# fcastagna/JoXSZ

Hardware: AMD Instinct MI355X
Metric: walker-likelihoods/sec at 512^2 map, 500-pt grid (higher is better)
Workload: dtype f64; 1 GPU; 1024 walkers/GPU, 512x512 SZ map, 500-pt radial grid, joint X-ray+SZ likelihood, synthetic CL J1226.9+3332-shaped inputs (BASELINE configs[2]); walkers_per_gpu=1024, S=512, N=500, B=55, chunk=1024, route=map, conv=custom, form=exact, sampling=none, radial_sampling=none, truncation=none, parallelism=walkers sharded x1, device=AMD GPU (gfx950:sramecc+:xnack-, 256 CUs)

## Files before the change

### joxsz_amd/csrc/joxsz_hip.hip

```cpp
#include <dlfcn.h>
#include <unistd.h>

#include <cctype>

#include "jx_ctx.hpp"

static int g_rocfft_refs = 0;

static size_t tensor_bytes(const jx_config& c, int id) {
    const size_t f = sizeof(double);
    switch (id) {
        case JX_T_R_PP: return f * c.N;
        case JX_T_D_MAT: return f * (size_t)c.S * c.S;
        case JX_T_BEAM_2D: return f * (size_t)c.B * c.B;
        case JX_T_FILTERING: return f * (size_t)c.S * c.S;
        case JX_T_RADIUS: return f * c.S;
        case JX_T_FLUX_DATA: return f * 3 * c.nflux;
        case JX_T_CONV_T: case JX_T_CONV_V: return f * c.nconv;
        case JX_T_PAR_VALS: case JX_T_PAR_MIN: case JX_T_PAR_MAX: case JX_T_PAR_MU: case JX_T_PAR_SIGMA:
            return f * c.npar;
        case JX_T_PAR_KIND: return sizeof(int32_t) * c.npar;
        case JX_T_THAWED_IDX: return sizeof(int32_t) * c.ndim;
        case JX_T_X_R_NE: case JX_T_X_R_T: case JX_T_GEOMAREA: return f * c.nann;
        case JX_T_PROJVOLS: return f * (size_t)c.nann * c.nann;
// ... 71 lines not shown
    if (d.quad) {
        d.pairw = 2;
        if (map_lds_need(d, threads) > (LDS_MAX - 2048) / 2) d.pairw = 1;
    } else if (pair_full && d.fast_map) {
        d.pairw = 2;
        if (map_lds_need(d, threads) > LDS_MAX - 1024) d.pairw = 1;
    }
    while (threads > 64 && map_lds_need(d, threads) > LDS_MAX - 1024) threads /= 2;
    const size_t lds = map_lds_need(d, threads);
    if (lds > LDS_MAX - 1024) return false;
    *threads_out = threads; *lds_out = lds;
    return true;
}

static void launch_map(hipStream_t st, const JxDev& dm_in, int threads, size_t lds, const double* theta_dev, int w0, int n, double* img,
                       double* tpp, double* tab, double* ty, bool coef_only) {
    JxDev dm = dm_in;
    dm.nlaunch = n;
    const bool vec2 = (dm.S % 2 == 0) && (dm.img_ld % 2 == 0);
    const int npw = (dm.pairw == 2) ? 2 : 1;
    if (coef_only) dm.map_split = 1;
    const dim3 grid(((n + npw - 1) / npw) * dm.map_split), block(threads);
    if (dm.fast_map) {
        const int nait = (dm.q_na + 63) / 64;
#define JX_SYM_LAUNCH(V, NA) hipLaunchKernelGGL((jx_abel_map_sym_kernel<V, NA>), grid, block, lds, st, dm, theta_dev, w0, img, tpp, tab, ty)
        if (vec2) { if (nait <= 3) JX_SYM_LAUNCH(true, 3); else if (nait <= 5) JX_SYM_LAUNCH(true, 5); else JX_SYM_LAUNCH(true, 9); }
        else      { if (nait <= 3) JX_SYM_LAUNCH(false, 3); else if (nait <= 5) JX_SYM_LAUNCH(false, 5); else JX_SYM_LAUNCH(false, 9); }
#undef JX_SYM_LAUNCH
    } else {
        if (vec2) hipLaunchKernelGGL(jx_abel_map_kernel<true>, grid, block, lds, st, dm, theta_dev, w0, img, tpp, tab, ty);
        else hipLaunchKernelGGL(jx_abel_map_kernel<false>, grid, block, lds, st, dm, theta_dev, w0, img, tpp, tab, ty);
    }
}

static int launch_y2d(jx_ctx* ctx, const Chunk& c) {
    int rc;
    if (!ctx->d_img && (rc = dev_new(ctx, (size_t)ctx->chunk * c.d.img_ws, &ctx->d_img, true))) return rc;
    launch_map(c.st, ctx->d, ctx->map_threads, ctx->map_lds, c.theta, c.w0, c.n, ctx->d_img, nullptr, nullptr, nullptr, false);
    return JX_OK;
}

static bool prep_splits(const jx_ctx* ctx, const Chunk& c) {
    const JxDev& d = c.d;
    return ctx->prep_split && !c.t.any() && !d.sz_only && !d.prep_pow && !d.calc_integ  && 3 * d.nann <= 128 && d.nband * d.nann <= 4096 && d.N <= 640;
}

#ifdef JOXSZ_ABLATIONS
static void prep_stamps(hipStream_t ps, int n, bool xr_split, JxDev& dp) {
    static long long* stamps = nullptr;
    if (!stamps) { (void)hipMalloc((void**)&stamps, sizeof(long long) * 8 * 65536); (void)hipMemset(stamps, 0, sizeof(long long) * 8 * 65536); }
    dp.stamps = stamps;
    static int calls = 0;
    if (++calls != 40) return;
    (void)hipStreamSynchronize(ps);
    const int nb = xr_split ? 2 * n : n;
    std::vector<long long> h((size_t)nb * 8);
    (void)hipMemcpy(h.data(), stamps, sizeof(long long) * h.size(), hipMemcpyDeviceToHost);
    long long t0 = h[0];
    for (int b = 0; b < nb; ++b) t0 = std::min(t0, h[(size_t)b * 8]);
    for (int half = 0; half < (xr_split ? 2 : 1); ++half) {
        const int b0 = half * n, b1 = b0 + n;
        double mx[7] = {0}, sm[7] = {0};
        for (int b = b0; b < b1; ++b)
            for (int k = 0; k < 7; ++k) { const double v = h[(size_t)b * 8 + k] ? (h[(size_t)b * 8 + k] - t0) * 0.01 : 0.0; mx[k] = std::max(mx[k], v); sm[k] += v / n; }
        fprintf(stderr, "prep stamps, %s blocks (us after the first start; mean/max): start %.2f/%.2f params %.2f/%.2f priors %.2f/%.2f grid pass %.2f/%.2f veto+integ %.2f/%.2f factors %.2f/%.2f end %.2f/%.2f\n",
                half ? "X-ray" : (xr_split ? "SZ-side" : "all"), sm[0], mx[0], sm[1], mx[1], sm[2], mx[2], sm[3], mx[3], sm[4], mx[4], sm[5], mx[5], sm[6], mx[6]);
    }
}
#endif

static void launch_prep(jx_ctx* ctx, const Chunk& c, hipStream_t ps, double* pp_buf, int pp_ld, int ncf) {
    const JxDev& d = c.d;
    const Taps& t = c.t;
    const int n = c.n;
    JxDev dp = d;
    dp.inject_pp = ctx->d.inject_pp;
    dp.xr_split = c.xr_split ? 1 : 0;
    dp.xr_out = ctx->d_xr;
    dp.pp_ld = pp_ld;
#ifdef JOXSZ_ABLATIONS
    if (opt_str(ctx, "JOXSZ_P_STAMPS")) prep_stamps(ps, n, c.xr_split, dp);
#endif
    const unsigned pgrid = c.xr_split ? 2u * (unsigned)n : (unsigned)n, pthr = c.xr_split ? 128u : (unsigned)JX_PREP_THREADS;
    if (c.xr_split && ctx->prep_lean && ctx->prep_fastmath && pp_buf && sizeof(double) * JX_W2_LDS_DOUBLES(d) <= (size_t)19 * 1024 + 512) {
        hipLaunchKernelGGL(jx_walker2_kernel, dim3(pgrid), dim3(JX_W2_THREADS), sizeof(double) * JX_W2_LDS_DOUBLES(d), ps, dp, c.theta, c.w0, c.base, c.cfac, pp_buf, ncf, c.sm);
        return;
    }
    const size_t sh = sizeof(double) * (JX_LDS_HDR + (size_t)2 * d.N + 2 * d.nann + 2 * (size_t)d.nband * d.nann + 2 * (size_t)d.nconv + 8 + JX_FM_TABLE_DOUBLES);
    if (d.prep_pow) hipLaunchKernelGGL((jx_prep_kernel<true, false>), dim3(pgrid), dim3(pthr), sh, ps, dp, c.theta, c.w0,
                                       c.base, c.cfac, pp_buf, c.sz0, t.tprof, t.xprofs, t.parts, t.integ, c.sm);
    else if (ctx->prep_fastmath) hipLaunchKernelGGL((jx_prep_kernel<false, true>), dim3(pgrid), dim3(pthr), sh, ps, dp, c.theta, c.w0,
                                                    c.base, c.cfac, pp_buf, c.sz0, t.tprof, t.xprofs, t.parts, t.integ, c.sm);
    else hipLaunchKernelGGL((jx_prep_kernel<false, false>), dim3(pgrid), dim3(pthr), sh, ps, dp, c.theta, c.w0,
                            c.base, c.cfac, pp_buf, c.sz0, t.tprof, t.xprofs, t.parts, t.integ, c.sm);
}

#include "jx_host_fft.hpp"
#include "jx_host_mix.hpp"
#include "jx_host_exact.hpp"

extern "C" {

int jx_comm_unique_id(void* id_out) {
    if (!id_out) return JX_ERR_INVALID;
    if (!rccl_load()) { g_last_global_error = g_rccl.err; return JX_ERR_COMM; }
    ncclUniqueId id;
    const ncclResult_t r = g_rccl.GetUniqueId(&id);
    if (r != ncclSuccess) { g_last_global_error = std::string("ncclGetUniqueId: ") + g_rccl.GetErrorString(r); return JX_ERR_COMM; }
    static_assert(sizeof(id) == JX_COMM_ID_BYTES, "id size");
    memcpy(id_out, &id, sizeof(id));
    return JX_OK;
}

int jx_comm_init_rank(jx_ctx* ctx, const void* idp, int nranks, int rank) {
    if (!ctx || !idp || nranks < 1 || rank < 0 || rank >= nranks) return JX_ERR_INVALID;
    if (ctx->comm) { ctx->err = "jx_comm_init_rank: this context already has a communicator"; return JX_ERR_STATE; }
    if (!rccl_load()) { ctx->err = g_rccl.err; return JX_ERR_COMM; }
    HIPCHK(ctx, hipSetDevice(ctx->cfg.device));
    ncclUniqueId id;
    memcpy(&id, idp, sizeof(id));
    fflush(stdout);
    const int saved = dup(1);
    if (saved >= 0) dup2(2, 1);
    const ncclResult_t r0 = g_rccl.CommInitRank(&ctx->comm, nranks, id, rank);
    fflush(stdout);
    if (saved >= 0) { dup2(saved, 1); close(saved); }
    NCCLCHK(ctx, r0);
    ctx->comm_rank = rank; ctx->comm_size = nranks;
    return JX_OK;
}

int jx_comm_count(jx_ctx* ctx) {
    if (!ctx) return JX_ERR_INVALID;
    if (!ctx->comm) { ctx->err = "jx_comm_count before jx_comm_init_rank"; return JX_ERR_STATE; }
    int n = 0;
    NCCLCHK(ctx, g_rccl.CommCount(ctx->comm, &n));
    return n;
}

static int gather_drain(jx_ctx* ctx) {
    for (auto& pr : ctx->gt_inflight) {
        HIPCHK(ctx, hipEventSynchronize(pr.second));
        float ms = 0.f;
        HIPCHK(ctx, hipEventElapsedTime(&ms, pr.first, pr.second));
        ctx->gather_ms += ms; ctx->gather_calls += 1;
        ctx->gt_free.push_back(pr);
    }
    ctx->gt_inflight.clear();
    return JX_OK;
}

static int comm_fork(jx_ctx* ctx, hipStream_t* out) {
    if (!ctx->comm_overlap) { *out = ctx->stream; return JX_OK; }
    HIPCHK(ctx, hipEventRecord(ctx->ev_fork, ctx->stream));
    HIPCHK(ctx, hipStreamWaitEvent(ctx->comm_stream, ctx->ev_fork, 0));
    *out = ctx->comm_stream;
    return JX_OK;
}

int jx_comm_set_overlap(jx_ctx* ctx, int on) {
    if (!ctx) return JX_ERR_INVALID;
    HIPCHK(ctx, hipSetDevice(ctx->cfg.device));
    HIPCHK(ctx, hipStreamSynchronize(ctx->stream));
    if (ctx->comm_stream) HIPCHK(ctx, hipStreamSynchronize(ctx->comm_stream));
    if (on && !ctx->comm_stream) {
        HIPCHK(ctx, hipStreamCreateWithFlags(&ctx->comm_stream, hipStreamNonBlocking));
        HIPCHK(ctx, hipEventCreateWithFlags(&ctx->ev_fork, hipEventDisableTiming));
// ... 347 lines not shown
            jxt::abel_matrix(r, A);
            for (int i = 0; i < N; ++i) {
                const double f = d.y_scale * wy[i];
                for (int j = i; j < N; ++j) wp[j] += f * A[(size_t)i * N + j];
            }
            if ((rc = dev_put(ctx, wp.data(), wp.size(), &p))) return rc;
            d.integ_wp = p; d.calc_integ = 1; d.integ_mu = c.integ_mu; d.integ_sig = c.integ_sig;
        }
    }
    {
        std::vector<double> rt(r.begin(), r.begin() + ctx->nt), G;
        if (!jxt::mirrored_spline_op(rt, G)) { ctx->err = "h(0) operator: singular system"; return JX_ERR_INVALID; }
        std::vector<double>& hw = h_hw;
        hw.assign(ctx->nt, 0.0);
        for (int j = 0; j < ctx->nt; ++j) hw[j] = -0.5 * rt[0] * rt[0] * G[j];
        hw[0] += 1.0;
        double* p; if ((rc = dev_put(ctx, hw.data(), hw.size(), &p))) return rc; d.hw = p;
    }
    {
        double* p; if ((rc = dev_put(ctx, h_E.data(), h_E.size(), &p))) return rc; d.emat = p;
        if ((rc = dev_put(ctx, h_flux.data(), h_flux.size(), &p))) return rc; d.flux = p;
    }
    {
        double* p;
        std::vector<double> tw((size_t)S * 2);
        for (int m = 0; m < S; ++m) { tw[2 * m] = std::cos(2.0 * jxt::kPi * m / S); tw[2 * m + 1] = std::sin(2.0 * jxt::kPi * m / S); }
        if ((rc = dev_put(ctx, tw.data(), tw.size(), &p))) return rc; d.twid = p;
    }
    return JX_OK;
}

static int walker_tables(jx_ctx* ctx, const std::vector<double>& r, const std::vector<double>& h_hw) {
    const jx_config& c = ctx->cfg;
    JxDev& d = ctx->d;
    int rc;
    {
        double* p; int* q;
#define PUTD(field, id) { std::vector<double> v = host_vec<double>(ctx, id); if ((rc = dev_put(ctx, v.data(), v.size(), &p))) return rc; d.field = p; }
#define PUTI(field, id) { std::vector<int32_t> v = host_vec<int32_t>(ctx, id); if ((rc = dev_put(ctx, v.data(), v.size(), &q))) return rc; d.field = q; }
        {
            std::vector<double> lr = r;
            for (double& v : lr) v = std::log(v);
            if ((rc = dev_put(ctx, lr.data(), lr.size(), &p))) return rc;
            d.lr_pp = p;
        }
        {
            std::vector<double> fm;
            jxt::fastmath_tables(fm);
            if ((rc = dev_put(ctx, fm.data(), fm.size(), &p))) return rc;
            d.fm_tab = p;
        }
        PUTD(r_pp, JX_T_R_PP) PUTD(d_mat, JX_T_D_MAT) PUTD(conv_T, JX_T_CONV_T) PUTD(conv_v, JX_T_CONV_V)
        PUTD(par_vals, JX_T_PAR_VALS) PUTD(par_min, JX_T_PAR_MIN) PUTD(par_max, JX_T_PAR_MAX)
        PUTD(par_mu, JX_T_PAR_MU) PUTD(par_sigma, JX_T_PAR_SIGMA)
        {
            std::vector<double> sg = host_vec<double>(ctx, JX_T_PAR_SIGMA);
            for (double& v : sg) v = (v > 0.0) ? -0.5 * std::log(2.0 * 3.14159265358979323846) - std::log(v) : 0.0;
            if ((rc = dev_put(ctx, sg.data(), sg.size(), &p))) return rc;
            d.par_lnorm = p;
        }
        PUTI(par_kind, JX_T_PAR_KIND) PUTI(thawed_idx, JX_T_THAWED_IDX)
        ctx->d_par_vals = const_cast<double*>(d.par_vals);
        {
            std::vector<double> pack;
            jxt::fastmath_tables(pack);
            pack.insert(pack.end(), r.begin(), r.end());
            for (double v : r) pack.push_back(std::log(v));
            pack.insert(pack.end(), h_hw.begin(), h_hw.end());
            for (int id : {JX_T_CONV_T, JX_T_CONV_V}) { const std::vector<double> v = host_vec<double>(ctx, id); pack.insert(pack.end(), v.begin(), v.end()); }
            if (pack.size() != JX_SZ_PACK_DOUBLES(d)) { ctx->err = "per-walker table pack: size"; return JX_ERR_INVALID; }
            if ((rc = dev_put(ctx, pack.data(), pack.size(), &p))) return rc;
            d.sz_pack = p;
        }
        if (!c.sz_only) {
            PUTD(x_r_ne, JX_T_X_R_NE) PUTD(x_r_T, JX_T_X_R_T) PUTD(projvols, JX_T_PROJVOLS) PUTD(cts, JX_T_CTS)
            PUTD(areascales, JX_T_AREASCALES) PUTD(exposures, JX_T_EXPOSURES) PUTD(backrates, JX_T_BACKRATES)
            PUTD(geomarea, JX_T_GEOMAREA) PUTD(lnT, JX_T_LNT) PUTD(lnrate, JX_T_LNRATE)
            std::vector<double> pack;
            jxt::fastmath_tables(pack);
            for (int id : {JX_T_X_R_NE, JX_T_X_R_T, JX_T_GEOMAREA, JX_T_LNT, JX_T_PROJVOLS, JX_T_AREASCALES, JX_T_EXPOSURES, JX_T_BACKRATES, JX_T_CTS}) {
                const std::vector<double> v = host_vec<double>(ctx, id);
                pack.insert(pack.end(), v.begin(), v.end());
            }
            if (pack.size() != JX_XR_PACK_DOUBLES(d)) { ctx->err = "X-ray table pack: size"; return JX_ERR_INVALID; }
            if ((rc = dev_put(ctx, pack.data(), pack.size(), &p))) return rc;
            d.xr_pack = p;
        }
#undef PUTD
#undef PUTI
    }
    return JX_OK;
}

static int map_tables(jx_ctx* ctx, const std::vector<double>& r) {
    const jx_config& c = ctx->cfg;
    const int S = c.S, N = c.N;
    const std::vector<double>& Qtab = ctx->h_Qtab;
    JxDev& d = ctx->d;
    int rc;
    {
        const int na = ctx->qn;
        const bool sym = ctx->dmat_mirror && na <= 9 * 64;
        d.fast_map = sym ? 1 : 0;
        d.q_na = d.q_nb = na;
        if (sym) {
            std::vector<int32_t> qk((size_t)na * na);
            std::vector<double> qt((size_t)na * na);
            for (size_t e = 0; e < Qtab.size(); ++e) {
                const double dd = Qtab[e];
                if (!(dd <= r[N - 1])) { qk[e] = N; qt[e] = (dd != dd) ? dd : 0.0; }
                else if (dd < r[0]) { qk[e] = N - 1; qt[e] = dd; }
                else {
                    int k = (int)(std::upper_bound(r.begin(), r.end(), dd) - r.begin()) - 1;
                    k = std::max(0, std::min(N - 2, k));
                    qk[e] = k; qt[e] = dd - r[k];
                }
            }
            int* qi; double* qd;
            if ((rc = dev_put(ctx, qk.data(), qk.size(), &qi))) return rc; d.q_k = qi;
            if ((rc = dev_put(ctx, qt.data(), qt.size(), &qd))) return rc; d.q_t = qd;
        }
    }
    int split = c.map_split > 0 ? c.map_split : 1;
    if (const char* e = opt_str(ctx, "JOXSZ_MAP_SPLIT")) { int v = atoi(e); if (v > 0) split = v; }
    d.map_split = std::min(split, S);
    return JX_OK;
}

static int chunk_capacity(jx_ctx* ctx, int chunk, int P, size_t mix_doubles, bool contracted_planned) {
    const jx_config& c = ctx->cfg;
    const int S = c.S;
    JxDev& d = ctx->d;
    int rc;
    const size_t budget = (size_t)24 << 30;
    if (ctx->conv_mode == 2) {
        d.quad = 1;
        d.img_ld = (d.q_na + 16) & ~15; d.img_ws = (long long)d.q_nb * d.img_ld;
        const size_t per_walker = sizeof(double) * mix_doubles;
        if (c.max_batch <= 0 && !opt_str(ctx, "JOXSZ_CHUNK")) while (chunk > 128 && per_walker * chunk > budget) chunk /= 2;
    } else {
        d.quad = 0; d.img_ld = P; d.img_ws = (long long)P * P;
        const size_t per_walker = sizeof(double) * ((size_t)P * P * 2 + (size_t)P * d.Ph * 2 + (size_t)S * ctx->Sh * 2);
        while (chunk > 1 && per_walker * chunk > budget) chunk /= 2;
    }
    ctx->chunk = chunk;
    if (!map_geometry(d, 512, &ctx->map_threads, &ctx->map_lds)) {
        if (ctx->conv_mode != 2) { ctx->err = "radial grid too long for the LDS-resident spline of the Abel + map kernel (the rocFFT sequence needs it)"; return JX_ERR_UNSUPPORTED; }
        if (ctx->map_ok && contracted_planned) { ctx->err = "radial grid too long for the Abel + map kernel after the contracted tables were planned with it: use the exact form (JOXSZ_MIX_FORM=exact)"; return JX_ERR_UNSUPPORTED; }
        ctx->map_ok = false;
    }
    {
        const int lds = 160 * 1024 - 1024;
#define JX_ATTR(V, NA) HIPCHK(ctx, hipFuncSetAttribute((const void*)jx_abel_map_sym_kernel<V, NA>, hipFuncAttributeMaxDynamicSharedMemorySize, lds))
        JX_ATTR(true, 3); JX_ATTR(true, 5); JX_ATTR(true, 9); JX_ATTR(false, 3); JX_ATTR(false, 5); JX_ATTR(false, 9);
#undef JX_ATTR
        HIPCHK(ctx, hipFuncSetAttribute((const void*)jx_abel_map_kernel<true>, hipFuncAttributeMaxDynamicSharedMemorySize, lds));
        HIPCHK(ctx, hipFuncSetAttribute((const void*)jx_abel_map_kernel<false>, hipFuncAttributeMaxDynamicSharedMemorySize, lds));
    }
    if ((rc = dev_new(ctx, (size_t)chunk, &ctx->d_base))) return rc;
    if ((rc = dev_new(ctx, (size_t)chunk * 2, &ctx->d_xr))) return rc;
    if ((rc = dev_new(ctx, (size_t)chunk * ctx->nrow, &ctx->d_cfac))) return rc;
    if (c.calc_integ && (rc = dev_new(ctx, (size_t)chunk, &ctx->d_sz0, true))) return rc;
    return JX_OK;
}

static int finalize_impl(jx_ctx* ctx) {
    if (!ctx) return JX_ERR_INVALID;
    if (ctx->finalized) { ctx->err = "jx_finalize called twice"; return JX_ERR_STATE; }
    const jx_config& c = ctx->cfg;
// ... 943 lines not shown
```

### joxsz_amd/csrc/jx_kernels.hpp

```cpp
#pragma once
#include <hip/hip_runtime.h>
#include <type_traits>
#include "jx_fastmath.hpp"
#include <stdint.h>

#ifdef JOXSZ_ABLATIONS
#define JX_DBG(c, bits) ((c).dbg & (bits))
#else
#define JX_DBG(c, bits) false
#endif
#ifdef JOXSZ_ABLATIONS
#define JX_PSTAMP(c, k) do { if ((c).stamps && threadIdx.x == 0) (c).stamps[(size_t)blockIdx.x * 8 + (k)] = wall_clock64(); } while (0)
#else
#define JX_PSTAMP(c, k) do { } while (0)
#endif
#define JX_MAX_PAR 19
#define JX_LDS_DECL extern __shared__ __attribute__((aligned(16))) double sm[]
#define JX_LDS_HDR 32
#ifdef JX_PREP_THREADS_OVERRIDE
#define JX_PREP_THREADS JX_PREP_THREADS_OVERRIDE
#else
#define JX_PREP_THREADS 256
#endif
#define JX_TAIL_THREADS 256

enum {
    P_LOGN0 = 0, P_BETA, P_LOGRC, P_LOGRS, P_ALPHA, P_EPS, P_GAMMA, P_LOGTR, P_Z,
    P_P0, P_A, P_B, P_C, P_RP, P_BACKSCALE, P_CALIB, P_LOGN02, P_BETA2, P_LOGRC2
};

enum { REJ_BOX = 1, REJ_MASS = 2, REJ_RCRS = 4, REJ_XRAY = 8 };

struct JxDev {
    int S, N, B, P, Ph, Sh, nrow, nt, nflux, nconv, nann, nband, ntab, npar, ndim;
    int ne_mode, exclude_unphy_mass, sz_only;
    int K;
    int map_split;
    double y_scale;
    double inv_h_mean;
    double inv_dlnT;
    const double* r_pp;
    const double* d_mat;
    long long img_ld, img_ws;
    int dbg;
    const double* fm_tab;
    int xr_split;
    double* xr_out;
    int prep_pow;
    const double* lr_pp;
    const double* sz_pack;
    const double* xr_pack;
    const double* inject_pp;
    long long* stamps;
    int pp_ld;
    int fast_map, q_na, q_nb;
    double* xcol;
    long long xcol_ld;
    int pairw, nlaunch;
    int quad;
    int calc_integ;
    const double* integ_wp;
    double integ_mu, integ_sig;
    double* cf_out;
    long long cf_ws;
    int cf_tr;
    const int* q_k;
    const double* q_t;
    const double* abel_tab;
    const double* gband;
    const double* bhat;
    const double* htab;
    const double* twid;
    const double* hw;
    const double* emat;
    const double* flux;
    const double* conv_T; const double* conv_v;
    const double* par_vals; const double* par_min; const double* par_max;
    const double* par_mu; const double* par_sigma; const double* par_lnorm;
    const int* par_kind; const int* thawed_idx;
    const double* x_r_ne; const double* x_r_T; const double* projvols; const double* cts;
    const double* areascales; const double* exposures; const double* backrates;
    const double* geomarea; const double* lnT; const double* lnrate;
};


__device__ __forceinline__ double jx_press(const double* p, double r) {
    const double x = r / p[P_RP];
    return p[P_P0] / (pow(x, p[P_C]) * pow(1.0 + pow(x, p[P_A]), (p[P_B] - p[P_C]) / p[P_A]));
}

__device__ __forceinline__ void jx_ne_consts(const double* p, int mode, double* pc) {
    const double n0 = pow(10.0, p[P_LOGN0]);
    pc[0] = n0 * n0; pc[1] = pow(10.0, p[P_LOGRC]); pc[2] = pow(10.0, p[P_LOGRS]);
    const double n02 = (mode == 1) ? pow(10.0, p[P_LOGN02]) : 0.0;
    pc[3] = n02 * n02; pc[4] = (mode == 1) ? pow(10.0, p[P_LOGRC2]) : 1.0;
}
__device__ __forceinline__ double jx_ne_pc(const double* p, const double* pc, double r, int mode) {
    const double x = r / pc[1];
    double res = pc[0] * ((p[P_ALPHA] == 0.0) ? 1.0 : pow(x, -p[P_ALPHA])) /
                 (pow(1.0 + x * x, 3.0 * p[P_BETA] - p[P_ALPHA] / 2.0) *
                  pow(1.0 + pow(r / pc[2], p[P_GAMMA]), p[P_EPS] / p[P_GAMMA]));
    if (mode == 1) {
        const double x2 = r / pc[4];
        res += pc[3] / pow(1.0 + x2 * x2, 3.0 * p[P_BETA2]);
    }
    return sqrt(res);
}
// ... 146 lines not shown
template <int U>
__device__ __forceinline__ void jx_copy_batched(double* __restrict__ dst, const double* __restrict__ src, int n, int tid, int nth) {
    for (int i0 = 0; i0 < n; i0 += U * nth) {
        double v[U];
#pragma unroll
        for (int u = 0; u < U; ++u) v[u] = src[min(i0 + u * nth + tid, n - 1)];
#pragma unroll
        for (int u = 0; u < U; ++u) { const int i = i0 + u * nth + tid; if (i < n) dst[i] = v[u]; }
    }
}

template <bool POW, class M>
__device__ __forceinline__ void jx_xray_side(const JxDev& c, const JxXrTab& xt, const double* p, const double* pl, const double* pc, const M& mt, int tid, int nth,
                                             double* s_x, double* s_ne, double* s_T, double* s_rate, double* s_term, double* red, int* redi,
                                             size_t w, double* __restrict__ tap_xprofs, double* xlike_out, int* xbad_out) {
    constexpr bool logform = !POW;
    if (logform && 3 * c.nann <= nth) {
        const int grp = tid / c.nann, k = tid - grp * c.nann;
        if (grp < 3) {
            const double rn = xt.x_r_ne[k], r = xt.x_r_T[k];
            if (grp == 0) s_ne[k] = jx_ne_log(mt, p, pl, rn, mt.l(rn), c.ne_mode);
            else if (grp == 1) { double xa; s_T[k] = jx_press_log(mt, p, pl, mt.l(r), &xa) * mt.e(2.30258509299404568402 * p[P_LOGTR]); }
            else s_x[k] = (rn == r) ? 0.0 : jx_ne_log(mt, p, pl, r, mt.l(r), c.ne_mode);
        }
        __syncthreads();
        if (tid < c.nann) s_T[tid] = s_T[tid] / ((xt.x_r_ne[tid] == xt.x_r_T[tid]) ? s_ne[tid] : s_x[tid]);
    } else if (tid < c.nann) {
        const double rn = xt.x_r_ne[tid], r = xt.x_r_T[tid];
        if (logform) {
            double xa;
            const double lr = mt.l(r);
            s_ne[tid] = jx_ne_log(mt, p, pl, rn, (rn == r) ? lr : mt.l(rn), c.ne_mode);
            s_T[tid] = jx_press_log(mt, p, pl, lr, &xa) / jx_ne_log(mt, p, pl, r, lr, c.ne_mode) * mt.e(2.30258509299404568402 * p[P_LOGTR]);
        } else {
            s_ne[tid] = jx_ne_pc(p, pc, rn, c.ne_mode);
            s_T[tid] = jx_press(p, r) / jx_ne_pc(p, pc, r, c.ne_mode) * pow(10.0, p[P_LOGTR]);
        }
    }
    __syncthreads();
    JX_PSTAMP(c, 2);
    const int nba = c.nband * c.nann;
    for (int q = tid; q < nba; q += nth) {
        const int b = q / c.nann, j = q - b * c.nann;
        const double lt = mt.l(s_T[j]);
        const double* tab = xt.lnrate + (size_t)b * 2 * c.ntab;
        double i0, i1;
        jx_interp_clamped2(xt.lnT, tab, tab + c.ntab, c.ntab, lt, c.inv_dlnT, &i0, &i1);
        const double z0 = mt.e(i0), z1 = mt.e(i1);
        s_rate[q] = (z0 + (z1 - z0) * p[P_Z]) * s_ne[j] * s_ne[j];
    }
    __syncthreads();
    JX_PSTAMP(c, 3);
    int bad = 0;
    for (int q = tid; q < nba; q += nth) {
        const int b = q / c.nann, i = q - b * c.nann;
        double proj = 0.0;
        for (int j = 0; j < c.nann; ++j) proj += xt.projvols[i * c.nann + j] * s_rate[b * c.nann + j];
        const double ae = xt.areascales[q] * xt.exposures[q];
        const double model = proj * ae + xt.backrates[q] * xt.geomarea[i] * ae * p[P_BACKSCALE];
        if (tap_xprofs) tap_xprofs[w * nba + q] = model;
        if (!(model > 0.0)) bad = 1;
        const double ct = xt.cts[q];
        s_term[q] = (ct == ct) ? ct * mt.l(model) - model : 0.0;
    }
    JX_PSTAMP(c, 4);
    int xbad = jx_block_or(bad, redi);
    JX_PSTAMP(c, 5);
    if (tid < 64) {
        double tot = 0.0;
        for (int q0 = 0; q0 < nba; q0 += 64) {
            double v = (q0 + tid < nba) ? s_term[q0 + tid] : 0.0;
            for (int off = 32; off > 0; off >>= 1) v += __shfl_down(v, off, 64);
            tot += v;
        }
        if (tid == 0) red[0] = tot;
    }
    __syncthreads();
    const double xlike = red[0];
    __syncthreads();
    if (!(fabs(xlike) <= 1.79769313486231570e308)) xbad = 1;
    *xlike_out = xlike; *xbad_out = xbad;
}

template <bool POW, bool FM = false>
__global__ void __launch_bounds__(JX_PREP_THREADS) __attribute__((amdgpu_waves_per_eu(4, 4)))
jx_prep_kernel(JxDev c, const double* __restrict__ theta, int w0,
               double* __restrict__ base, double* __restrict__ cfac, double* __restrict__ pp_out ,
               double* __restrict__ sz0 ,
               double* __restrict__ tap_tprof, double* __restrict__ tap_xprofs, double* __restrict__ tap_parts, double* __restrict__ tap_integ,
               JxSm smv) {
    JX_LDS_DECL;
    double* p = sm;
    double* red = sm + 20;
    int& redi = *reinterpret_cast<int*>(sm + 28);
    const int nblk = c.xr_split ? (int)(gridDim.x >> 1) : (int)gridDim.x;
    const bool xonly = c.xr_split && (int)blockIdx.x >= nblk;
    const bool noxr = c.xr_split && !xonly;
    const int w = xonly ? (int)blockIdx.x - nblk : (int)blockIdx.x;
    const int gw = w0 + w;
    const int tid = threadIdx.x, nth = blockDim.x;
    JX_PSTAMP(c, 0);

    double* s_m = sm + JX_LDS_HDR;
    double* s_t = s_m + c.N;
    double* s_ne = s_t + c.N;
    double* s_T = s_ne + c.nann;
    double* s_rate = s_T + c.nann;
    double* s_conv = s_rate + c.nband * c.nann;
    double* s_fm = s_conv + 2 * c.nconv;
    double* s_term = s_fm + JX_FM_TABLE_DOUBLES;
    static_assert(!(POW && FM), "the tables serve the log form");
    typename std::conditional<FM, JxMathTab, JxMathLib>::type mt;
    if constexpr (FM) { mt.t.et = s_fm; mt.t.lt = s_fm + JX_FM_EXP_N; }

    const bool has_par = tid < c.npar;
    const int pk_kind = has_par ? c.par_kind[tid] : 0;
    const double pk_a = has_par ? (pk_kind == 1 ? c.par_mu[tid] : c.par_min[tid]) : 0.0;
    const double pk_b = has_par ? (pk_kind == 1 ? c.par_sigma[tid] : c.par_max[tid]) : 0.0;
    const double pk_ln = has_par ? c.par_lnorm[tid] : 0.0;
    for (int i = tid; i < 2 * c.nconv; i += nth) s_conv[i] = (i < c.nconv) ? c.conv_T[i] : c.conv_v[i - c.nconv];
    if (FM) for (int i = tid; i < JX_FM_TABLE_DOUBLES; i += nth) s_fm[i] = c.fm_tab[i];
    jx_load_params(c, theta, gw, p, &smv);
    JX_PSTAMP(c, 1);
    double pc[5] = {0, 1, 1, 0, 1};
    if (POW) jx_ne_consts(p, c.ne_mode, pc);

    constexpr bool logform = !POW;
    double pl[11];
    jx_prof_consts(mt, p, c.ne_mode, pl);
    double pr = 0.0, parprior = 0.0;
    int rej = 0;
    if (!xonly) {
    if (has_par) {
        const double v = p[tid];
        if (pk_kind == 1) {
            const double sg = pk_b;
            if (sg <= 0.0) { rej |= REJ_BOX; }
            else {
                const double z = (v - pk_a) / sg;
                pr = pk_ln - 0.5 * z * z;
            }
        } else if (v < pk_a || v > pk_b) rej |= REJ_BOX;
        if (v != v) rej |= REJ_BOX;
    }
    parprior = jx_block_sum(pr, red);
    JX_PSTAMP(c, 2);
    if (!(fabs(parprior) <= 1.79769313486231570e308)) rej |= REJ_BOX;

    if (tid == 0 && (POW ? (pow(10.0, p[P_LOGRC]) > pow(10.0, p[P_LOGRS])) : (p[P_LOGRC] > p[P_LOGRS]))) rej |= REJ_RCRS;

    const bool veto = c.exclude_unphy_mass != 0;
    const int nprof = (veto || pp_out || c.calc_integ) ? c.N : c.nt;
    double ci = 0.0;
    const int nt_ = c.nt, mode_ = c.ne_mode;
    const size_t ppo = (size_t)w * (c.pp_ld ? c.pp_ld : c.N);
    if (logform) {
        for (int i = tid; i < nprof; i += 2 * nth) {
            const int i2 = min(i + nth, nprof - 1);
            const bool two = i + nth < nprof;
            const double ra = c.r_pp[i], rb = c.r_pp[i2], lra = c.lr_pp[i], lrb = c.lr_pp[i2];
            double xaa, xab;
            const double pa = jx_press_log(mt, p, pl, lra, &xaa), pb = jx_press_log(mt, p, pl, lrb, &xab);
            const double ia = jx_inv_ne_log(mt, p, pl, ra, lra, mode_), ib = jx_inv_ne_log(mt, p, pl, rb, lrb, mode_);
            const double ma = pa * (p[P_C] + p[P_B] * xaa) * ra * ia / (1.0 + xaa);
            const double mb = pb * (p[P_C] + p[P_B] * xab) * rb * ib / (1.0 + xab);
            if (pp_out) { pp_out[ppo + i] = pa; if (two) pp_out[ppo + i2] = pb; }
            if (c.calc_integ) { ci = fma(c.integ_wp[i], pa, ci); if (two) ci = fma(c.integ_wp[i2], pb, ci); }
            if (veto) { s_m[i] = ma; if (two) s_m[i2] = mb; }
            if (i < nt_) s_t[i] = pa * ia;
            if (two && i2 < nt_) s_t[i2] = pb * ib;
        }
    } else {
        for (int i = tid; i < nprof; i += nth) {
            const double r = c.r_pp[i];
            const double x = r / p[P_RP];
            const double xa = pow(x, p[P_A]);
            const double press = p[P_P0] / (pow(x, p[P_C]) * pow(1.0 + xa, (p[P_B] - p[P_C]) / p[P_A]));
            if (pp_out) pp_out[ppo + i] = press;
            if (c.calc_integ) ci = fma(c.integ_wp[i], press, ci);
            if (veto || i < nt_) {
                const double ne = jx_ne_pc(p, pc, r, mode_);
                if (veto) s_m[i] = press * (p[P_C] + p[P_B] * xa) / (r * (1.0 + xa)) * r * r / ne;
                if (i < nt_) s_t[i] = press / ne;
            }
        }
    }
    __syncthreads();
    JX_PSTAMP(c, 3);
    if (veto) {
        for (int i = tid; i < c.N; i += nth) {
            double g;
            if (i == 0) g = s_m[1] - s_m[0];
            else if (i == c.N - 1) g = s_m[c.N - 1] - s_m[c.N - 2];
            else g = (s_m[i + 1] - s_m[i - 1]) / 2.0;
            if (!(g > 0.0)) rej |= REJ_MASS;
        }
    }

    if (c.calc_integ) {
        const double cint = jx_block_sum(ci, red);
        if (tid == 0) {
            const double z = (cint - c.integ_mu) / c.integ_sig;
            const double z2 = z * z;
            if (sz0) sz0[w] = (z2 == z2) ? -0.5 * z2 : 0.0;
            if (tap_integ) tap_integ[w] = cint;
        }
    }

    JX_PSTAMP(c, 4);
    double part = 0.0;
    for (int k = tid; k < c.nt; k += nth) part += c.hw[k] * s_t[k];
    const double t0 = jx_block_sum(part, red);
    for (int k = tid; k < c.nrow; k += nth) {
        const double T = (k == 0) ? t0 : s_t[k - 1];
        cfac[(size_t)w * c.nrow + k] = jx_convert_tab(s_conv, s_conv + c.nconv, c.nconv, T) * p[P_CALIB];
        if (tap_tprof) tap_tprof[(size_t)w * c.nrow + k] = T;
    }
    __syncthreads();
    JX_PSTAMP(c, 5);
    }

    double xlike = 0.0;
    int xbad = 0;
    if (!c.sz_only && !noxr) {
        const JxXrTab xt{c.x_r_ne, c.x_r_T, c.lnT, c.lnrate, c.projvols, c.areascales, c.exposures, c.backrates, c.geomarea, c.cts};
        jx_xray_side<POW>(c, xt, p, pl, pc, mt, tid, nth, s_m, s_ne, s_T, s_rate, s_term, red, &redi, (size_t)w, tap_xprofs, &xlike, &xbad);
        if (xbad) rej |= REJ_XRAY;
    }
    if (xonly) {
        if (tid == 0) { c.xr_out[2 * (size_t)w] = xlike; c.xr_out[2 * (size_t)w + 1] = xbad ? 1.0 : 0.0; }
        JX_PSTAMP(c, 6);
        return;
    }
    const int rejall = jx_block_or(rej, &redi);
    if (tid == 0) {
        double prior = parprior;
        double b = (rejall != 0) ? -INFINITY : (prior + xlike);
        base[w] = b;
        if (tap_parts) {
            tap_parts[(size_t)w * 4 + 0] = (rejall & REJ_XRAY) ? -INFINITY : xlike;
            tap_parts[(size_t)w * 4 + 2] = (rejall & (REJ_BOX | REJ_RCRS)) ? -INFINITY : prior;
            tap_parts[(size_t)w * 4 + 3] = (double)rejall;
        }
    }
    JX_PSTAMP(c, 6);
}

#define JX_W2_THREADS 128
#define JX_SZ_PACK_DOUBLES(c) ((size_t)JX_FM_TABLE_DOUBLES + 2 * (size_t)(c).N + (c).nt + 2 * (size_t)(c).nconv)
#define JX_XR_PACK_DOUBLES(c) ((size_t)JX_FM_TABLE_DOUBLES + 3 * (size_t)(c).nann + (c).ntab + (size_t)(c).nann * (c).nann + 4 * (size_t)(c).nband * (c).nann)
#define JX_W2_LDS_DOUBLES(c) (JX_LDS_HDR + ((JX_SZ_PACK_DOUBLES(c) + (size_t)(c).N + (c).nt) > (JX_XR_PACK_DOUBLES(c) + 3 * (size_t)(c).nann + 2 * (size_t)(c).nband * (c).nann) \
                                             ? (JX_SZ_PACK_DOUBLES(c) + (size_t)(c).N + (c).nt) : (JX_XR_PACK_DOUBLES(c) + 3 * (size_t)(c).nann + 2 * (size_t)(c).nband * (c).nann)) + 8)

__global__ void __launch_bounds__(JX_W2_THREADS) __attribute__((amdgpu_waves_per_eu(4, 4)))
jx_walker2_kernel(JxDev c, const double* __restrict__ theta, int w0, double* __restrict__ base, double* __restrict__ cfac, double* __restrict__ pp_out,
                  int ncf , JxSm smv) {
    JX_LDS_DECL;
    double* p = sm;
    double* red = sm + 20;
    int& redi = *reinterpret_cast<int*>(sm + 28);
    const int nblk = (int)(gridDim.x >> 1);
    const bool xonly = (int)blockIdx.x >= nblk;
    const int w = xonly ? (int)blockIdx.x - nblk : (int)blockIdx.x, gw = w0 + w;
    const int tid = threadIdx.x, nth = JX_W2_THREADS;
    JX_PSTAMP(c, 0);
    double* s_pack = sm + JX_LDS_HDR;
    JxMathTab mt;
    mt.t.et = s_pack; mt.t.lt = s_pack + JX_FM_EXP_N;
    if (xonly) {
        jx_copy_batched<12>(s_pack, c.xr_pack, (int)JX_XR_PACK_DOUBLES(c), tid, nth);
        jx_load_params(c, theta, gw, p, &smv);
        JX_PSTAMP(c, 1);
        const int nann = c.nann, nba = c.nband * c.nann;
        const double* t = s_pack + JX_FM_TABLE_DOUBLES;
        const JxXrTab xt{t, t + nann, t + 3 * nann, c.lnrate, t + 3 * nann + c.ntab, t + 3 * nann + c.ntab + nann * nann, t + 3 * nann + c.ntab + nann * nann + nba,
                         t + 3 * nann + c.ntab + nann * nann + 2 * nba, t + 2 * nann, t + 3 * nann + c.ntab + nann * nann + 3 * nba};
        double* s_ne = s_pack + JX_XR_PACK_DOUBLES(c);
        double* s_T = s_ne + nann;
        double* s_x = s_T + nann;
        double* s_rate = s_x + nann;
        double* s_term = s_rate + nba;
        double pl[11];
        jx_prof_consts(mt, p, c.ne_mode, pl);
        const double pc[5] = {0, 1, 1, 0, 1};
        double xlike = 0.0;
        int xbad = 0;
        jx_xray_side<false>(c, xt, p, pl, pc, mt, tid, nth, s_x, s_ne, s_T, s_rate, s_term, red, &redi, (size_t)w, nullptr, &xlike, &xbad);
        if (tid == 0) { c.xr_out[2 * (size_t)w] = xlike; c.xr_out[2 * (size_t)w + 1] = xbad ? 1.0 : 0.0; }
        JX_PSTAMP(c, 6);
        return;
    }
    const int N = c.N, nt = c.nt;
    const double* s_r = s_pack + JX_FM_TABLE_DOUBLES;
    const double* s_lr = s_r + N;
    const double* s_hw = s_lr + N;
    const double* s_conv = s_hw + nt;
    double* s_m = s_pack + JX_SZ_PACK_DOUBLES(c);
    double* s_t = s_m + N;
    const bool has_par = tid < c.npar;
    const int pk_kind = has_par ? c.par_kind[tid] : 0;
    const double pk_a = has_par ? (pk_kind == 1 ? c.par_mu[tid] : c.par_min[tid]) : 0.0;
    const double pk_b = has_par ? (pk_kind == 1 ? c.par_sigma[tid] : c.par_max[tid]) : 0.0;
    const double pk_ln = has_par ? c.par_lnorm[tid] : 0.0;
    jx_copy_batched<20>(s_pack, c.sz_pack, (int)JX_SZ_PACK_DOUBLES(c), tid, nth);
    jx_load_params(c, theta, gw, p, &smv);
    JX_PSTAMP(c, 1);
    double pl[11];
    jx_prof_consts(mt, p, c.ne_mode, pl);
    double pr = 0.0;
    int rej = 0;
    if (has_par) {
        const double v = p[tid];
        if (pk_kind == 1) {
            const double sg = pk_b;
            if (sg <= 0.0) { rej |= REJ_BOX; }
            else {
                const double z = (v - pk_a) / sg;
                pr = pk_ln - 0.5 * z * z;
            }
        } else if (v < pk_a || v > pk_b) rej |= REJ_BOX;
        if (v != v) rej |= REJ_BOX;
    }
    const double parprior = jx_block_sum(pr, red);
    JX_PSTAMP(c, 2);
    if (!(fabs(parprior) <= 1.79769313486231570e308)) rej |= REJ_BOX;
    if (tid == 0 && p[P_LOGRC] > p[P_LOGRS]) rej |= REJ_RCRS;
    const bool veto = c.exclude_unphy_mass != 0;
    const int mode_ = c.ne_mode;
    const size_t ppo = (size_t)w * (c.pp_ld ? c.pp_ld : N);
    for (int i = tid; i < N; i += 2 * nth) {
        const int i2 = min(i + nth, N - 1);
        const bool two = i + nth < N;
        const double ra = s_r[i], rb = s_r[i2], lra = s_lr[i], lrb = s_lr[i2];
        double xaa, xab;
        const double pa = jx_press_log(mt, p, pl, lra, &xaa), pb = jx_press_log(mt, p, pl, lrb, &xab);
        const double ia = jx_inv_ne_log(mt, p, pl, ra, lra, mode_), ib = jx_inv_ne_log(mt, p, pl, rb, lrb, mode_);
        const double ma = pa * (p[P_C] + p[P_B] * xaa) * ra * ia / (1.0 + xaa);
        const double mb = pb * (p[P_C] + p[P_B] * xab) * rb * ib / (1.0 + xab);
        pp_out[ppo + i] = pa; if (two) pp_out[ppo + i2] = pb;
        if (veto) { s_m[i] = ma; if (two) s_m[i2] = mb; }
        if (i < nt) s_t[i] = pa * ia;
        if (two && i2 < nt) s_t[i2] = pb * ib;
    }
    __syncthreads();
    JX_PSTAMP(c, 3);
    if (veto) {
        for (int i = tid; i < N; i += nth) {
            double g;
            if (i == 0) g = s_m[1] - s_m[0];
            else if (i == N - 1) g = s_m[N - 1] - s_m[N - 2];
            else g = (s_m[i + 1] - s_m[i - 1]) / 2.0;
            if (!(g > 0.0)) rej |= REJ_MASS;
        }
    }
    JX_PSTAMP(c, 4);
    double part = 0.0;
    for (int k = tid; k < nt; k += nth) part += s_hw[k] * s_t[k];
    const double t0 = jx_block_sum(part, red);
    for (int k = tid; k < ncf; k += nth) {
        const double T = (k == 0) ? t0 : s_t[k - 1];
        cfac[(size_t)w * c.nrow + k] = jx_convert_tab(s_conv, s_conv + c.nconv, c.nconv, T) * p[P_CALIB];
    }
    JX_PSTAMP(c, 5);
    const int rejall = jx_block_or(rej, &redi);
    if (tid == 0) base[w] = (rejall != 0) ? -INFINITY : (parprior + 0.0);
    JX_PSTAMP(c, 6);
}

template <bool POW>
__global__ void __launch_bounds__(128)
jx_pp_kernel(JxDev c, const double* __restrict__ theta, int w0, double* __restrict__ pp_out ) {
    JX_LDS_DECL;
    double* p = sm;
    const int w = blockIdx.x, tid = threadIdx.x, nth = blockDim.x;
    jx_load_params(c, theta, w0 + w, p);
    const int N_ = c.N;
    double* __restrict__ out = pp_out + (size_t)w * N_;
    if (POW) {
        for (int i = tid; i < N_; i += nth) out[i] = jx_press(p, c.r_pp[i]);
    } else {
        double pl[11];
        const JxMathLib mt;
        jx_prof_consts(mt, p, c.ne_mode, pl);
        for (int i = tid; i < N_; i += 2 * nth) {
            const int i2 = min(i + nth, N_ - 1);
            double xa, xb;
            const double pa = jx_press_log(mt, p, pl, c.lr_pp[i], &xa), pb = jx_press_log(mt, p, pl, c.lr_pp[i2], &xb);
            out[i] = pa;
            if (i + nth < N_) out[i2] = pb;
        }
    }
}

__device__ __forceinline__ double jx_rsqrt(double x) {
    const double y0 = __builtin_amdgcn_rsq(x);
    const double e = fma(-x * y0, y0, 1.0);
    return fma(y0 * e, fma(e, 0.375, 0.5), y0);
}

__device__ __forceinline__ double jx_abel_row(const double2* s_rq, double ri2, int j0, int N) {
    double a0 = 0.0, a1 = 0.0, a2 = 0.0, a3 = 0.0;
    int j = j0;
    for (; j + 12 < N; j += 16) {
        const double2 q0 = s_rq[j], q1 = s_rq[j + 4], q2 = s_rq[j + 8], q3 = s_rq[j + 12];
        const double t0 = jx_rsqrt(q0.x - ri2), t1 = jx_rsqrt(q1.x - ri2), t2 = jx_rsqrt(q2.x - ri2), t3 = jx_rsqrt(q3.x - ri2);
        a0 = fma(q0.y, t0, a0); a1 = fma(q1.y, t1, a1); a2 = fma(q2.y, t2, a2); a3 = fma(q3.y, t3, a3);
    }
    for (; j < N; j += 4) {
        const double2 q0 = s_rq[j];
        a0 = fma(q0.y, jx_rsqrt(q0.x - ri2), a0);
    }
    return (a0 + a1) + (a2 + a3);
}

__device__ __forceinline__ void jx_profile_to_coefs(const JxDev& c, const double* p, int w, bool taps, double* s_r,
                                                    double* s_pp, double* s_y, double* s_M, double* s_cf, double2* s_rq,
                                                    double2* s_ds, double* tap_pp, double* tap_ab, double* tap_y) {
    const int N = c.N, tid = threadIdx.x, nth = blockDim.x;
    for (int j = tid; j < N; j += nth) {
        const double2 t0 = *reinterpret_cast<const double2*>(c.abel_tab + 4 * (size_t)j);
        const double2 t1 = *reinterpret_cast<const double2*>(c.abel_tab + 4 * (size_t)j + 2);
        const double r = t0.x;
        s_r[j] = r;
        s_ds[j] = t1;
        const double v = c.inject_pp ? c.inject_pp[(size_t)w * N + j] : (JX_DBG(c, 32) ? r : jx_press(p, r));
        s_pp[j] = v;
        s_rq[j] = make_double2(r * r, t0.y * v);
        if (taps && tap_pp) tap_pp[(size_t)w * N + j] = v;
    }
    __syncthreads();

    const int npair = (N + 1) >> 1;
    for (int p0 = 0; p0 < npair; p0 += (nth >> 2)) {
        const int pr = p0 + (tid >> 2), sub = tid & 3;
        double acc1 = 0.0, acc2 = 0.0;
        const int i1 = pr, i2 = N - 1 - pr;
        if (pr < npair && !JX_DBG(c, 8)) {
            if (JX_DBG(c, 128)) {
                const double ri1 = s_rq[i1].x, ri2 = s_rq[i2].x;
                for (int j = i1 + 2 + sub; j < N; j += 4) { const double2 q = s_rq[j]; acc1 = fma(q.y, q.x - ri1, acc1); }
                for (int j = i2 + 2 + sub; j < N; j += 4) { const double2 q = s_rq[j]; acc2 = fma(q.y, q.x - ri2, acc2); }
            } else {
                acc1 = jx_abel_row(s_rq, s_rq[i1].x, i1 + 2 + sub, N);
                if (i2 != i1) acc2 = jx_abel_row(s_rq, s_rq[i2].x, i2 + 2 + sub, N);
            }
        }
        acc1 += __shfl_xor(acc1, 1, 64); acc1 += __shfl_xor(acc1, 2, 64);
        acc2 += __shfl_xor(acc2, 1, 64); acc2 += __shfl_xor(acc2, 2, 64);
// ... 949 lines not shown
```

Baseline: 26.94 million walker-likelihoods/s.

## Lean walker2 prep: register-held radii, fused reductions, precomputed X-ray log radii

Reworks the split walker prep kernel. The SZ half now reads r and log r straight into registers instead of staging them in LDS, and copies only the remaining tables with 16-byte loads. Its three block reductions (prior sum, temperature sum, reject OR) are merged into one wave-shuffle pass with a single barrier. The X-ray half uses a new lean routine that gets log radii from a table precomputed once at setup, spreads the profile evaluations across thread groups, and reduces with fewer barriers. The intent is to cut LDS traffic, barrier count and repeated log evaluations per walker. The cost is added guards on N and nann (N at most 768, nann limited by thread count) and an extra setup kernel.

```diff
diff --git a/joxsz_amd/csrc/joxsz_hip.hip b/joxsz_amd/csrc/joxsz_hip.hip
--- a/joxsz_amd/csrc/joxsz_hip.hip
+++ b/joxsz_amd/csrc/joxsz_hip.hip
@@ -177,7 +177,8 @@
     if (opt_str(ctx, "JOXSZ_P_STAMPS")) prep_stamps(ps, n, c.xr_split, dp);
 #endif
     const unsigned pgrid = c.xr_split ? 2u * (unsigned)n : (unsigned)n, pthr = c.xr_split ? 128u : (unsigned)JX_PREP_THREADS;
-    if (c.xr_split && ctx->prep_lean && ctx->prep_fastmath && pp_buf && sizeof(double) * JX_W2_LDS_DOUBLES(d) <= (size_t)19 * 1024 + 512) {
+    if (c.xr_split && ctx->prep_lean && ctx->prep_fastmath && pp_buf && sizeof(double) * JX_W2_LDS_DOUBLES(d) <= (size_t)19 * 1024 + 512 &&
+        d.N <= JX_W2_RPL * JX_W2_THREADS && 3 * d.nann <= JX_W2_THREADS) {
         hipLaunchKernelGGL(jx_walker2_kernel, dim3(pgrid), dim3(JX_W2_THREADS), sizeof(double) * JX_W2_LDS_DOUBLES(d), ps, dp, c.theta, c.w0, c.base, c.cfac, pp_buf, ncf, c.sm);
         return;
     }
@@ -691,9 +692,13 @@
                 const std::vector<double> v = host_vec<double>(ctx, id);
                 pack.insert(pack.end(), v.begin(), v.end());
             }
+            pack.insert(pack.end(), 2 * (size_t)d.nann, 0.0);
             if (pack.size() != JX_XR_PACK_DOUBLES(d)) { ctx->err = "X-ray table pack: size"; return JX_ERR_INVALID; }
             if ((rc = dev_put(ctx, pack.data(), pack.size(), &p))) return rc;
             d.xr_pack = p;
+            hipLaunchKernelGGL(jx_xr_logr_kernel, dim3(1), dim3(64), 0, 0, d.fm_tab, p + JX_FM_TABLE_DOUBLES, p + pack.size() - 2 * (size_t)d.nann, 2 * d.nann);
+            HIPCHK(ctx, hipGetLastError());
+            HIPCHK(ctx, hipDeviceSynchronize());
         }
 #undef PUTD
 #undef PUTI
diff --git a/joxsz_amd/csrc/jx_kernels.hpp b/joxsz_amd/csrc/jx_kernels.hpp
--- a/joxsz_amd/csrc/jx_kernels.hpp
+++ b/joxsz_amd/csrc/jx_kernels.hpp
@@ -23,6 +23,7 @@
 #define JX_PREP_THREADS 256
 #endif
 #define JX_TAIL_THREADS 256
+#define JX_W2_THREADS 128
 
 enum {
     P_LOGN0 = 0, P_BETA, P_LOGRC, P_LOGRS, P_ALPHA, P_EPS, P_GAMMA, P_LOGTR, P_Z,
@@ -335,6 +336,129 @@
     *xlike_out = xlike; *xbad_out = xbad;
 }
 
+template <int U>
+__device__ __forceinline__ void jx_copy_batched16(double* __restrict__ dst, const double* __restrict__ src, int n, int split, int gap, int tid, int nth) {
+    const double2* __restrict__ s2 = reinterpret_cast<const double2*>(src);
+    double2* __restrict__ d2 = reinterpret_cast<double2*>(dst);
+    const int n2 = n >> 1, split2 = split >> 1, gap2 = gap >> 1;
+    for (int i0 = 0; i0 < n2; i0 += U * nth) {
+        double2 v[U];
+#pragma unroll
+        for (int u = 0; u < U; ++u) { const int i = min(i0 + u * nth + tid, n2 - 1); v[u] = s2[i < split2 ? i : i + gap2]; }
+#pragma unroll
+        for (int u = 0; u < U; ++u) { const int i = i0 + u * nth + tid; if (i < n2) d2[i] = v[u]; }
+    }
+    if ((n & 1) && tid == 0) dst[n - 1] = src[(n - 1 < split) ? n - 1 : n - 1 + gap];
+}
+
+template <class M>
+__device__ __forceinline__ void jx_xray_side_lean(const JxDev& c, const JxXrTab& xt, const double* xt_lr, const double* p, const double* pl, const M& mt, int tid,
+                                                  double* s_x, double* s_ne, double* s_T, double* s_rate, double* s_term, int* redw,
+                                                  size_t w) {
+    constexpr int nth = JX_W2_THREADS;
+    const int nann = c.nann;
+    if (2 * nann <= 64) {
+        if (tid < 64) {
+            const int second = tid >= nann, k = second ? tid - nann : tid;
+            if (tid < 2 * nann) {
+                const double rn = xt.x_r_ne[k], rT = xt.x_r_T[k];
+                const double r = second ? rT : rn, lr = xt_lr[tid];
+                double v = 0.0;
+                if (!(second && rn == rT)) v = jx_ne_log(mt, p, pl, r, lr, c.ne_mode);
+                (second ? s_x : s_ne)[k] = v;
+            }
+        } else if (tid - 64 < nann) {
+            double xa;
+            s_T[tid - 64] = jx_press_log(mt, p, pl, xt_lr[nann + tid - 64], &xa) * mt.e(2.30258509299404568402 * p[P_LOGTR]);
+        }
+    } else {
+        const int grp = tid / nann, k = tid - grp * nann;
+        if (grp < 3) {
+            const double rn = xt.x_r_ne[k], r = xt.x_r_T[k];
+            if (grp == 0) s_ne[k] = jx_ne_log(mt, p, pl, rn, xt_lr[k], c.ne_mode);
+            else if (grp == 1) { double xa; s_T[k] = jx_press_log(mt, p, pl, xt_lr[nann + k], &xa) * mt.e(2.30258509299404568402 * p[P_LOGTR]); }
+            else s_x[k] = (rn == r) ? 0.0 : jx_ne_log(mt, p, pl, r, xt_lr[nann + k], c.ne_mode);
+        }
+    }
+    __syncthreads();
+    if (tid < nann) {
+        const double T = s_T[tid] / ((xt.x_r_ne[tid] == xt.x_r_T[tid]) ? s_ne[tid] : s_x[tid]);
+        const double x = mt.l(T);
+        const double* xp = xt.lnT;
+        const int n = c.ntab;
+        int lo;
+        if (x != x) lo = -1;
+        else if (x <= xp[0]) lo = -2;
+        else if (x >= xp[n - 1]) lo = -3;
+        else {
+            lo = (int)((x - xp[0]) * c.inv_dlnT);
+            lo = max(0, min(n - 2, lo));
+            while (lo > 0 && xp[lo] > x) --lo;
+            while (lo < n - 2 && xp[lo + 1] <= x) ++lo;
+        }
+        s_T[tid] = x; reinterpret_cast<int*>(s_x)[2 * tid] = lo;
+    }
+    __syncthreads();
+    JX_PSTAMP(c, 2);
+    const int nba = c.nband * nann;
+    for (int q = tid; q < nba; q += nth) {
+        const int b = q / nann, j = q - b * nann;
+        const double x = s_T[j];
+        const int lo = reinterpret_cast<const int*>(s_x)[2 * j], n = c.ntab;
+        const double* f0 = xt.lnrate + (size_t)b * 2 * n;
+        const double* f1 = f0 + n;
+        double i0, i1;
+        if (lo == -1) { i0 = x; i1 = x; }
+        else if (lo == -2) { i0 = f0[0]; i1 = f1[0]; }
+        else if (lo == -3) { i0 = f0[n - 1]; i1 = f1[n - 1]; }
+        else {
+            const double* xp = xt.lnT;
+            const int hi = lo + 1;
+            const double dx = xp[hi] - xp[lo], t = x - xp[lo];
+            i0 = (f0[hi] - f0[lo]) / dx * t + f0[lo];
+            i1 = (f1[hi] - f1[lo]) / dx * t + f1[lo];
+        }
+        const double z0 = mt.e(i0), z1 = mt.e(i1);
+        s_rate[q] = (z0 + (z1 - z0) * p[P_Z]) * s_ne[j] * s_ne[j];
+    }
+    __syncthreads();
+    JX_PSTAMP(c, 3);
+    int bad = 0;
+    for (int q = tid; q < nba; q += nth) {
+        const int b = q / nann, i = q - b * nann;
+        double proj = 0.0;
+        for (int j = 0; j < nann; ++j) proj += xt.projvols[i * nann + j] * s_rate[b * nann + j];
+        const double ae = xt.areascales[q] * xt.exposures[q];
+        const double model = proj * ae + xt.backrates[q] * xt.geomarea[i] * ae * p[P_BACKSCALE];
+        if (!(model > 0.0)) bad = 1;
+        const double ct = xt.cts[q];
+        s_term[q] = (ct == ct) ? ct * mt.l(model) - model : 0.0;
+    }
+    JX_PSTAMP(c, 4);
+    const int wbad = __any(bad);
+    if ((tid & 63) == 0) redw[tid >> 6] = wbad;
+    __syncthreads();
+    JX_PSTAMP(c, 5);
+    if (tid < 64) {
+        double tot = 0.0;
+        for (int q0 = 0; q0 < nba; q0 += 64) {
+            double v = (q0 + tid < nba) ? s_term[q0 + tid] : 0.0;
+            for (int off = 32; off > 0; off >>= 1) v += __shfl_down(v, off, 64);
+            tot += v;
+        }
+        if (tid == 0) {
+            const int xbad = (redw[0] | redw[1]) || !(fabs(tot) <= 1.79769313486231570e308);
+            c.xr_out[2 * w] = tot; c.xr_out[2 * w + 1] = xbad ? 1.0 : 0.0;
+        }
+    }
+}
+
+__global__ void jx_xr_logr_kernel(const double* __restrict__ fm_tab, const double* __restrict__ r, double* __restrict__ out, int n) {
+    JxFm t;
+    t.et = fm_tab; t.lt = fm_tab + JX_FM_EXP_N;
+    for (int i = threadIdx.x; i < n; i += blockDim.x) out[i] = jx_fm_log(t, r[i]);
+}
+
 template <bool POW, bool FM = false>
 __global__ void __launch_bounds__(JX_PREP_THREADS) __attribute__((amdgpu_waves_per_eu(4, 4)))
 jx_prep_kernel(JxDev c, const double* __restrict__ theta, int w0,
@@ -499,11 +623,13 @@
     JX_PSTAMP(c, 6);
 }
 
-#define JX_W2_THREADS 128
+#define JX_W2_RPL 6
 #define JX_SZ_PACK_DOUBLES(c) ((size_t)JX_FM_TABLE_DOUBLES + 2 * (size_t)(c).N + (c).nt + 2 * (size_t)(c).nconv)
-#define JX_XR_PACK_DOUBLES(c) ((size_t)JX_FM_TABLE_DOUBLES + 3 * (size_t)(c).nann + (c).ntab + (size_t)(c).nann * (c).nann + 4 * (size_t)(c).nband * (c).nann)
-#define JX_W2_LDS_DOUBLES(c) (JX_LDS_HDR + ((JX_SZ_PACK_DOUBLES(c) + (size_t)(c).N + (c).nt) > (JX_XR_PACK_DOUBLES(c) + 3 * (size_t)(c).nann + 2 * (size_t)(c).nband * (c).nann) \
-                                             ? (JX_SZ_PACK_DOUBLES(c) + (size_t)(c).N + (c).nt) : (JX_XR_PACK_DOUBLES(c) + 3 * (size_t)(c).nann + 2 * (size_t)(c).nband * (c).nann)) + 8)
+#define JX_SZ_TAB_DOUBLES(c) ((size_t)JX_FM_TABLE_DOUBLES + (c).nt + 2 * (size_t)(c).nconv)
+#define JX_XR_PACK_DOUBLES(c) ((size_t)JX_FM_TABLE_DOUBLES + 5 * (size_t)(c).nann + (c).ntab + (size_t)(c).nann * (c).nann + 4 * (size_t)(c).nband * (c).nann)
+#define JX_W2_LDS_SZ(c) (JX_SZ_TAB_DOUBLES(c) + (size_t)(c).N + (c).nt)
+#define JX_W2_LDS_XR(c) (JX_XR_PACK_DOUBLES(c) + 3 * (size_t)(c).nann + 2 * (size_t)(c).nband * (c).nann)
+#define JX_W2_LDS_DOUBLES(c) (JX_LDS_HDR + (JX_W2_LDS_SZ(c) > JX_W2_LDS_XR(c) ? JX_W2_LDS_SZ(c) : JX_W2_LDS_XR(c)) + 8)
 
 __global__ void __launch_bounds__(JX_W2_THREADS) __attribute__((amdgpu_waves_per_eu(4, 4)))
 jx_walker2_kernel(JxDev c, const double* __restrict__ theta, int w0, double* __restrict__ base, double* __restrict__ cfac, double* __restrict__ pp_out,
@@ -511,7 +637,7 @@
     JX_LDS_DECL;
     double* p = sm;
     double* red = sm + 20;
-    int& redi = *reinterpret_cast<int*>(sm + 28);
+    int* redw = reinterpret_cast<int*>(sm + 24);
     const int nblk = (int)(gridDim.x >> 1);
     const bool xonly = (int)blockIdx.x >= nblk;
     const int w = xonly ? (int)blockIdx.x - nblk : (int)blockIdx.x, gw = w0 + w;
@@ -521,13 +647,14 @@
     JxMathTab mt;
     mt.t.et = s_pack; mt.t.lt = s_pack + JX_FM_EXP_N;
     if (xonly) {
-        jx_copy_batched<12>(s_pack, c.xr_pack, (int)JX_XR_PACK_DOUBLES(c), tid, nth);
+        jx_copy_batched16<6>(s_pack, c.xr_pack, (int)JX_XR_PACK_DOUBLES(c), 0, 0, tid, nth);
         jx_load_params(c, theta, gw, p, &smv);
         JX_PSTAMP(c, 1);
         const int nann = c.nann, nba = c.nband * c.nann;
         const double* t = s_pack + JX_FM_TABLE_DOUBLES;
         const JxXrTab xt{t, t + nann, t + 3 * nann, c.lnrate, t + 3 * nann + c.ntab, t + 3 * nann + c.ntab + nann * nann, t + 3 * nann + c.ntab + nann * nann + nba,
                          t + 3 * nann + c.ntab + nann * nann + 2 * nba, t + 2 * nann, t + 3 * nann + c.ntab + nann * nann + 3 * nba};
+        const double* s_lr = t + 3 * nann + c.ntab + nann * nann + 4 * nba;
         double* s_ne = s_pack + JX_XR_PACK_DOUBLES(c);
         double* s_T = s_ne + nann;
         double* s_x = s_T + nann;
@@ -535,27 +662,28 @@
         double* s_term = s_rate + nba;
         double pl[11];
         jx_prof_consts(mt, p, c.ne_mode, pl);
-        const double pc[5] = {0, 1, 1, 0, 1};
-        double xlike = 0.0;
-        int xbad = 0;
-        jx_xray_side<false>(c, xt, p, pl, pc, mt, tid, nth, s_x, s_ne, s_T, s_rate, s_term, red, &redi, (size_t)w, nullptr, &xlike, &xbad);
-        if (tid == 0) { c.xr_out[2 * (size_t)w] = xlike; c.xr_out[2 * (size_t)w + 1] = xbad ? 1.0 : 0.0; }
+        jx_xray_side_lean(c, xt, s_lr, p, pl, mt, tid, s_x, s_ne, s_T, s_rate, s_term, redw, (size_t)w);
         JX_PSTAMP(c, 6);
         return;
     }
     const int N = c.N, nt = c.nt;
-    const double* s_r = s_pack + JX_FM_TABLE_DOUBLES;
-    const double* s_lr = s_r + N;
-    const double* s_hw = s_lr + N;
+    const double* s_hw = s_pack + JX_FM_TABLE_DOUBLES;
     const double* s_conv = s_hw + nt;
-    double* s_m = s_pack + JX_SZ_PACK_DOUBLES(c);
+    double* s_m = s_pack + JX_SZ_TAB_DOUBLES(c);
     double* s_t = s_m + N;
     const bool has_par = tid < c.npar;
     const int pk_kind = has_par ? c.par_kind[tid] : 0;
     const double pk_a = has_par ? (pk_kind == 1 ? c.par_mu[tid] : c.par_min[tid]) : 0.0;
     const double pk_b = has_par ? (pk_kind == 1 ? c.par_sigma[tid] : c.par_max[tid]) : 0.0;
     const double pk_ln = has_par ? c.par_lnorm[tid] : 0.0;
-    jx_copy_batched<20>(s_pack, c.sz_pack, (int)JX_SZ_PACK_DOUBLES(c), tid, nth);
+    double rq[JX_W2_RPL], lq[JX_W2_RPL];
+#pragma unroll
+    for (int u = 0; u < JX_W2_RPL; ++u) {
+        const int i = min(tid + u * nth, N - 1);
+        rq[u] = c.sz_pack[JX_FM_TABLE_DOUBLES + i];
+        lq[u] = c.sz_pack[JX_FM_TABLE_DOUBLES + N + i];
+    }
+    jx_copy_batched16<3>(s_pack, c.sz_pack, (int)JX_SZ_TAB_DOUBLES(c), JX_FM_TABLE_DOUBLES, 2 * N, tid, nth);
     jx_load_params(c, theta, gw, p, &smv);
     JX_PSTAMP(c, 1);
     double pl[11];
@@ -574,17 +702,18 @@
         } else if (v < pk_a || v > pk_b) rej |= REJ_BOX;
         if (v != v) rej |= REJ_BOX;
     }
-    const double parprior = jx_block_sum(pr, red);
     JX_PSTAMP(c, 2);
-    if (!(fabs(parprior) <= 1.79769313486231570e308)) rej |= REJ_BOX;
     if (tid == 0 && p[P_LOGRC] > p[P_LOGRS]) rej |= REJ_RCRS;
     const bool veto = c.exclude_unphy_mass != 0;
     const int mode_ = c.ne_mode;
     const size_t ppo = (size_t)w * (c.pp_ld ? c.pp_ld : N);
-    for (int i = tid; i < N; i += 2 * nth) {
+#pragma unroll
+    for (int u = 0; u < JX_W2_RPL; u += 2) {
+        const int i = tid + u * nth;
+        if (i >= N) break;
         const int i2 = min(i + nth, N - 1);
         const bool two = i + nth < N;
-        const double ra = s_r[i], rb = s_r[i2], lra = s_lr[i], lrb = s_lr[i2];
+        const double ra = rq[u], rb = rq[u + 1], lra = lq[u], lrb = lq[u + 1];
         double xaa, xab;
         const double pa = jx_press_log(mt, p, pl, lra, &xaa), pb = jx_press_log(mt, p, pl, lrb, &xab);
         const double ia = jx_inv_ne_log(mt, p, pl, ra, lra, mode_), ib = jx_inv_ne_log(mt, p, pl, rb, lrb, mode_);
@@ -609,14 +738,25 @@
     JX_PSTAMP(c, 4);
     double part = 0.0;
     for (int k = tid; k < nt; k += nth) part += s_hw[k] * s_t[k];
-    const double t0 = jx_block_sum(part, red);
+    for (int off = 32; off > 0; off >>= 1) {
+        pr += __shfl_down(pr, off, 64);
+        part += __shfl_down(part, off, 64);
+        rej |= __shfl_down(rej, off, 64);
+    }
+    if ((tid & 63) == 0) { red[tid >> 6] = pr; red[2 + (tid >> 6)] = part; redw[tid >> 6] = rej; }
+    __syncthreads();
+    double parprior = 0.0, t0 = 0.0;
+    for (int k = 0; k < JX_W2_THREADS / 64; ++k) { parprior += red[k]; t0 += red[2 + k]; }
     for (int k = tid; k < ncf; k += nth) {
         const double T = (k == 0) ? t0 : s_t[k - 1];
         cfac[(size_t)w * c.nrow + k] = jx_convert_tab(s_conv, s_conv + c.nconv, c.nconv, T) * p[P_CALIB];
     }
     JX_PSTAMP(c, 5);
-    const int rejall = jx_block_or(rej, &redi);
-    if (tid == 0) base[w] = (rejall != 0) ? -INFINITY : (parprior + 0.0);
+    if (tid == 0) {
+        int rejall = redw[0] | redw[1];
+        if (!(fabs(parprior) <= 1.79769313486231570e308)) rejall |= REJ_BOX;
+        base[w] = (rejall != 0) ? -INFINITY : (parprior + 0.0);
+    }
     JX_PSTAMP(c, 6);
 }
 
```

Result: faster. 28.50 million walker-likelihoods/s (median of 6 runs) (+5.8%).
